# microsoft/SpeechT5

Hardware: AMD Instinct MI355X
Metric: audio-sec/s fwd+bwd SpeechT5-Base (higher is better)
Workload: dtype bf16

## Files before the change

### speecht5_amd/csrc/gemm.hip

```cpp
#include <type_traits>
#include "common.h"
#include "stream_scratch.h"
#include "../../include/speecht5_hip.h"

namespace {

constexpr int BM = 128, BN = 128, NTHREADS = 256;
constexpr int TILE_BYTES = 128 * 128;
constexpr int EP_LD = 68;

struct OpAddr {
  long long ld, bstride, seg_stride;
  int rpb, seg;
  __device__ __forceinline__ long long outer(int idx) const {
    return rpb ? (long long)(idx / rpb) * bstride + (long long)(idx % rpb) * ld : (long long)idx * ld;
  }
  __device__ __forceinline__ long long inner(int idx) const {
    return seg ? (long long)(idx / seg) * seg_stride + (idx % seg) : (long long)idx;
  }
};
__device__ __forceinline__ OpAddr make_addr(long long ld, long long bstride, long long seg_stride, int rpb, int seg) {
  OpAddr a; a.ld = ld; a.bstride = bstride; a.seg_stride = seg_stride; a.rpb = rpb; a.seg = seg;
  return a;
}
// ... 768 lines not shown
  if (p.dropout_p > 0.f) f |= F_DROP;
  if (p.R.ptr) f |= F_RES;
  if (p.Cpre.ptr) f |= F_PRE;
  if (p.beta != 0.f) f |= F_BETA;
  switch (f) {
    case 0: case F_GELU | F_PRE: case F_DROP | F_RES: case F_DACT: case F_BETA: case F_RES: return f;
    default: break;
  }
  if (log_rt) fprintf(stderr, "st5_gemm rt-epilogue feat=%d act=%d M=%d N=%d K=%d batch=%d\n", f, p.act, p.M, p.N, p.K, p.batch);
  return -1;
}

template <int... FS> struct FeatSet {};
typedef FeatSet<0, F_GELU | F_PRE, F_DROP | F_RES, F_DACT, F_BETA, F_RES> NtFeats;
typedef FeatSet<0, F_BETA> TnFeats;
template <int... FS, typename Fn>
int with_feat(const int feat, FeatSet<FS...>, Fn&& fn) {
  int rc = ST5_OK;
  const bool hit = ((feat == FS && (rc = fn(std::integral_constant<int, FS>()), true)) || ...);
  return hit ? rc : fn(std::integral_constant<int, -1>());
}
typedef __attribute__((address_space(3))) void* lds_ptr_t;
typedef const __attribute__((address_space(1))) void* gbl_ptr_t;

#ifndef GEMM_ABL
#define GEMM_ABL 0
#endif
#ifdef GEMM_TIMING
__device__ unsigned long long g_gemm_timing[8];
#define GPROBE(i) do { __builtin_amdgcn_s_waitcnt(0xC07F); const unsigned long long t_ = __builtin_amdgcn_s_memtime(); tacc[i] += (unsigned int)(t_ - tprev); tprev = t_; } while (0)
#else
#define GPROBE(i)
#endif

template <typename F, int OFF>
__device__ __forceinline__ F lds_read128_asm(const unsigned lds_addr) {
  static_assert(sizeof(F) == 16, "128-bit fragment");
  F v;
  asm volatile("ds_read_b128 %0, %1 offset:%2" : "=v"(v) : "v"(lds_addr), "n"(OFF) : "memory");
  return v;
}

#ifndef GLDS_AUX_A
#define GLDS_AUX_A 0
#endif
#ifndef GLDS_AUX_B
#define GLDS_AUX_B 0
#endif
template <typename T, int NBUF, int FEAT = -1>
__global__ __launch_bounds__(NTHREADS, 2) void gemm_nt_glds_kernel(const st5_gemm_params p, const int c_vec_ok) {
  if (st5_gate_dropped(p.gate)) return;
  ST5_PAD_TO_256_VGPRS();
#ifdef GEMM_TIMING
  unsigned int tacc[8] = {0, 0, 0, 0, 0, 0, 0, 0};
  unsigned long long tprev = __builtin_amdgcn_s_memtime();
#endif
  constexpr int VEC = Elem<T>::VEC;
  constexpr int BK = 128 / (int)sizeof(T);
  typedef typename Frag<T>::type frag_t;
  extern __shared__ __attribute__((aligned(16))) char dsm[];

  const int tid = threadIdx.x, lane = tid & 63, wave = tid >> 6;
  const int wr = wave >> 1, wc = wave & 1;
  const int z = blockIdx.z;
  const int tiles_n = (p.N + BN - 1) / BN;
// ... 3 lines not shown
  const int m0 = tm * BM, n0 = tn * BN;
  const T* Ap = reinterpret_cast<const T*>(p.A.ptr) + z_off(p.A.zs0, p.A.zs1, z, p.zdiv);
  const T* Bp = reinterpret_cast<const T*>(p.B.ptr) + z_off(p.B.zs0, p.B.zs1, z, p.zdiv);
  const OpAddr aa = make_addr(p.A.ld, p.A.bstride, 0, p.A.rpb, 0);
  const OpAddr ab = make_addr(p.B.ld, p.B.bstride, 0, p.B.rpb, 0);

  const T* asrc[4];
  const T* bsrc[4];
  const int rsub = lane >> 3, pc = lane & 7;
#pragma unroll
  for (int i = 0; i < 4; ++i) {
    const int row = (i * 4 + wave) * 8 + rsub;
    const int c = pc ^ ((row >> 1) & 7);
    int gr = m0 + row; gr = gr < p.M ? gr : p.M - 1;
    asrc[i] = Ap + aa.outer(gr) + c * VEC;
    int gc = n0 + row; gc = gc < p.N ? gc : p.N - 1;
    bsrc[i] = Bp + ab.outer(gc) + c * VEC;
  }
  const int dst0 = wave * 1024;

  auto issue = [&](int kt, int buf) {
    char* base = dsm + buf * 2 * TILE_BYTES + dst0;
#pragma unroll
    for (int i = 0; i < 4; ++i) {
      __builtin_amdgcn_global_load_lds((gbl_ptr_t)(asrc[i] + (long long)kt * BK), (lds_ptr_t)(base + i * 4096), 16, 0, GLDS_AUX_A);
      __builtin_amdgcn_global_load_lds((gbl_ptr_t)(bsrc[i] + (long long)kt * BK), (lds_ptr_t)(base + TILE_BYTES + i * 4096), 16, 0, GLDS_AUX_B);
    }
  };
  auto issue_a = [&](int kt, int slot) {
    char* base = dsm + slot * TILE_BYTES + dst0;
#pragma unroll
    for (int i = 0; i < 4; ++i)
      __builtin_amdgcn_global_load_lds((gbl_ptr_t)(asrc[i] + (long long)kt * BK), (lds_ptr_t)(base + i * 4096), 16, 0, GLDS_AUX_A);
  };
  auto issue_b = [&](int kt, int slot) {
    char* base = dsm + slot * TILE_BYTES + dst0;
#pragma unroll
    for (int i = 0; i < 4; ++i)
      __builtin_amdgcn_global_load_lds((gbl_ptr_t)(bsrc[i] + (long long)kt * BK), (lds_ptr_t)(base + i * 4096), 16, 0, GLDS_AUX_B);
  };

  f32x16 acc00, acc01, acc10, acc11;
#pragma unroll
  for (int r = 0; r < 16; ++r) { acc00[r] = 0.f; acc01[r] = 0.f; acc10[r] = 0.f; acc11[r] = 0.f; }

  const int nk = p.K / BK;
  if constexpr (NBUF == 5) {
    issue_a(0, 0); issue_b(0, 1);
    if (nk > 1) issue_a(1, 2);
  } else {
#pragma unroll
    for (int t = 0; t < NBUF - 1; ++t)
      if (t < nk) issue(t, t);
  }
  const int frow = lane & 31, fhalf = lane >> 5;
  const int arow0 = wr * 64 + frow, brow0 = wc * 64 + frow;
  const unsigned lds_base = (unsigned)(size_t)(lds_ptr_t)dsm;
  const unsigned a_addr0 = lds_off(arow0, fhalf), b_addr0 = lds_off(brow0, fhalf);
  GPROBE(0);
  int sa = 0;
  for (int kt = 0; kt < nk; ++kt) {
    if constexpr (NBUF == 5) {
      if (kt + 1 < nk) asm volatile("s_waitcnt vmcnt(4)" ::: "memory");
      else asm volatile("s_waitcnt vmcnt(0)" ::: "memory");
    } else {
      int ahead = nk - 1 - kt;
      ahead = ahead < NBUF - 2 ? ahead : NBUF - 2;
      if (ahead >= 3) asm volatile("s_waitcnt vmcnt(24)" ::: "memory");
      else if (ahead == 2) asm volatile("s_waitcnt vmcnt(16)" ::: "memory");
      else if (ahead == 1) asm volatile("s_waitcnt vmcnt(8)" ::: "memory");
      else asm volatile("s_waitcnt vmcnt(0)" ::: "memory");
    }
    __builtin_amdgcn_s_barrier();
    GPROBE(1);
#if GEMM_ABL != 2
    if constexpr (NBUF == 5) {
      if (kt + 1 < nk) issue_b(kt + 1, sa + 3 >= 5 ? sa - 2 : sa + 3);
      if (kt + 2 < nk) issue_a(kt + 2, sa + 4 >= 5 ? sa - 1 : sa + 4);
    } else {
      if (kt + NBUF - 1 < nk) issue(kt + NBUF - 1, (kt + NBUF - 1) % NBUF);
    }
#endif
    unsigned pa, pb;
    if constexpr (NBUF == 5) {
      const int sb = sa + 1 >= 5 ? 0 : sa + 1;
      pa = lds_base + sa * TILE_BYTES + a_addr0; pb = lds_base + sb * TILE_BYTES + b_addr0;
      sa = sa + 2 >= 5 ? sa - 3 : sa + 2;
    } else {
      const unsigned cb = lds_base + (kt % NBUF) * 2 * TILE_BYTES;
      pa = cb + a_addr0; pb = cb + TILE_BYTES + b_addr0;
    }
    frag_t fa0[2], fa1[2], fb0[2], fb1[2];
#define NT_READ(S, KG)                                                                                      \
  fa0[S] = lds_read128_asm<frag_t, 0>(pa ^ ((KG) << 5)); fb0[S] = lds_read128_asm<frag_t, 0>(pb ^ ((KG) << 5));          \
  fa1[S] = lds_read128_asm<frag_t, 4096>(pa ^ ((KG) << 5)); fb1[S] = lds_read128_asm<frag_t, 4096>(pb ^ ((KG) << 5));
#define NT_WAIT(S, CNT)                                                                                     \
  asm volatile("s_waitcnt lgkmcnt(" #CNT ")" : "+v"(fa0[S]), "+v"(fa1[S]), "+v"(fb0[S]), "+v"(fb1[S]) :: "memory");
#if GEMM_ABL == 3
#define NT_MMA(S) asm volatile("" :: "v"(fa0[S]), "v"(fa1[S]), "v"(fb0[S]), "v"(fb1[S]));
#else
#define NT_MMA(S)                                                                                           \
  mma<T>(fa0[S], fb0[S], acc00); mma<T>(fa0[S], fb1[S], acc01); mma<T>(fa1[S], fb0[S], acc10); mma<T>(fa1[S], fb1[S], acc11);
#endif
    NT_READ(0, 0)
    NT_READ(1, 1)
    NT_WAIT(0, 4)
    NT_MMA(0) __builtin_amdgcn_sched_barrier(0);
    NT_READ(0, 2)
    NT_WAIT(1, 4)
    NT_MMA(1) __builtin_amdgcn_sched_barrier(0);
    NT_READ(1, 3)
    NT_WAIT(0, 4)
// ... 32 lines not shown
  float* stage = reinterpret_cast<float*>(dsm) + wave * (32 * EP_LD);
#if GEMM_ABL == 1
  asm volatile("" :: "v"(acc00), "v"(acc01), "v"(acc10), "v"(acc11));
  if (ea.alpha == 123.f)
#endif
  run_epilogue<T, FEAT>(ea, stage, acc00, acc01, acc10, acc11, m0 + wr * 64, n0 + wc * 64, lane);
#ifdef GEMM_TIMING
  GPROBE(4);
  if (lane == 0) { for (int i = 0; i < 5; ++i) atomicAdd(&g_gemm_timing[i], (unsigned long long)tacc[i]); atomicAdd(&g_gemm_timing[7], 1ull); }
#endif
}


constexpr int M64_A_BYTES = 64 * 128, M64_STAGE = M64_A_BYTES + TILE_BYTES;

template <int FEAT>
__global__ __launch_bounds__(NTHREADS, 3) void gemm_nt_m64_kernel(const st5_gemm_params p, const int c_vec_ok) {
  if (st5_gate_dropped(p.gate)) return;
  typedef bf16_t T;
  constexpr int VEC = 8, BK = 64;
  typedef bf16x8 frag_t;
  extern __shared__ __attribute__((aligned(16))) char dsm[];

  const int tid = threadIdx.x, lane = tid & 63, wave = tid >> 6;
  const int wr = wave >> 1, wc = wave & 1;
  const int z = blockIdx.z;
  const int tiles_n = (p.N + BN - 1) / BN;
  const int bid = xcd_remap((int)blockIdx.x, (int)gridDim.x);
  int tm, tn;
  tile_of(bid, tiles_n, (int)gridDim.x, tm, tn);
  const int m0 = tm * 64, n0 = tn * BN;
// ... 1 lines not shown
  const T* Bp = reinterpret_cast<const T*>(p.B.ptr) + z_off(p.B.zs0, p.B.zs1, z, p.zdiv);
  const OpAddr aa = make_addr(p.A.ld, p.A.bstride, 0, p.A.rpb, 0);
  const OpAddr ab = make_addr(p.B.ld, p.B.bstride, 0, p.B.rpb, 0);

  const T* asrc[2];
  const T* bsrc[4];
  const int rsub = lane >> 3, pc = lane & 7;
#pragma unroll
  for (int i = 0; i < 4; ++i) {
    const int row = (i * 4 + wave) * 8 + rsub;
    const int c = pc ^ ((row >> 1) & 7);
    if (i < 2) {
      int gr = m0 + row; gr = gr < p.M ? gr : p.M - 1;
      asrc[i] = Ap + aa.outer(gr) + c * VEC;
    }
    int gc = n0 + row; gc = gc < p.N ? gc : p.N - 1;
    bsrc[i] = Bp + ab.outer(gc) + c * VEC;
  }
  const int dst0 = wave * 1024;
  auto issue = [&](int kt, int buf) {
    char* base = dsm + buf * M64_STAGE + dst0;
#pragma unroll
    for (int i = 0; i < 2; ++i)
      __builtin_amdgcn_global_load_lds((gbl_ptr_t)(asrc[i] + (long long)kt * BK), (lds_ptr_t)(base + i * 4096), 16, 0, 0);
#pragma unroll
    for (int i = 0; i < 4; ++i)
      __builtin_amdgcn_global_load_lds((gbl_ptr_t)(bsrc[i] + (long long)kt * BK), (lds_ptr_t)(base + M64_A_BYTES + i * 4096), 16, 0, 0);
  };

  f32x16 acc0, acc1;
#pragma unroll
  for (int r = 0; r < 16; ++r) { acc0[r] = 0.f; acc1[r] = 0.f; }

  const int nk = p.K / BK;
  issue(0, 0);
  const int frow = lane & 31, fhalf = lane >> 5;
  const unsigned lds_base = (unsigned)(size_t)(lds_ptr_t)dsm;
  const unsigned a_addr0 = lds_off(wr * 32 + frow, fhalf), b_addr0 = M64_A_BYTES + lds_off(wc * 64 + frow, fhalf);
  for (int kt = 0; kt < nk; ++kt) {
    asm volatile("s_waitcnt vmcnt(0)" ::: "memory");
    __builtin_amdgcn_s_barrier();
    if (kt + 1 < nk) issue(kt + 1, (kt + 1) & 1);
    const unsigned cb = lds_base + (kt & 1) * M64_STAGE;
    const unsigned pa = cb + a_addr0, pb = cb + b_addr0;
    frag_t fa[2], fb0[2], fb1[2];
#define M64_READ(S, KG)                                                                                     \
  fa[S] = lds_read128_asm<frag_t, 0>(pa ^ ((KG) << 5)); fb0[S] = lds_read128_asm<frag_t, 0>(pb ^ ((KG) << 5));           \
  fb1[S] = lds_read128_asm<frag_t, 4096>(pb ^ ((KG) << 5));
#define M64_WAIT(S, CNT)                                                                                    \
  asm volatile("s_waitcnt lgkmcnt(" #CNT ")" : "+v"(fa[S]), "+v"(fb0[S]), "+v"(fb1[S]) :: "memory");
#define M64_MMA(S) mma<T>(fa[S], fb0[S], acc0); mma<T>(fa[S], fb1[S], acc1);
    M64_READ(0, 0)
    M64_READ(1, 1)
    M64_WAIT(0, 3)
    M64_MMA(0) __builtin_amdgcn_sched_barrier(0);
    M64_READ(0, 2)
    M64_WAIT(1, 3)
    M64_MMA(1) __builtin_amdgcn_sched_barrier(0);
    M64_READ(1, 3)
    M64_WAIT(0, 3)
    M64_MMA(0) __builtin_amdgcn_sched_barrier(0);
    M64_WAIT(1, 0)
    M64_MMA(1) __builtin_amdgcn_sched_barrier(0);
#undef M64_READ
#undef M64_WAIT
// ... 190 lines not shown
      if (ea.out_f32) ea.R = reinterpret_cast<const float*>(ea.R) + zr; else ea.R = reinterpret_cast<const T*>(ea.R) + zr;
    }
    if (ea.P) ea.P = reinterpret_cast<const T*>(ea.P) + z_off(p.P.zs0, p.P.zs1, z, p.zdiv);
    if (ea.Cpre) ea.Cpre = reinterpret_cast<T*>(ea.Cpre) + z_off(p.Cpre.zs0, p.Cpre.zs1, z, p.zdiv);
  }
  float* stage = reinterpret_cast<float*>(dsm) + wave * (32 * EP_LD);
  run_epilogue<T>(ea, stage, acc[0][0], acc[0][1], acc[1][0], acc[1][1], m0 + wr * 128, n0 + wc * 64, lane);
  run_epilogue<T>(ea, stage, acc[2][0], acc[2][1], acc[3][0], acc[3][1], m0 + wr * 128 + 64, n0 + wc * 64, lane);
#ifdef GEMM_TIMING
  GPROBE(4);
  if (lane == 0) { for (int i = 0; i < 5; ++i) atomicAdd(&g_gemm_timing[i], (unsigned long long)tacc[i]); atomicAdd(&g_gemm_timing[7], 1ull); }
#endif
}


template <int FEAT, bool STAGGER>
__global__ __launch_bounds__(512) void gemm_nt8p_kernel(const st5_gemm_params p, const int c_vec_ok) {
  if (st5_gate_dropped(p.gate)) return;
  typedef bf16_t T;
  constexpr int BK = 64;
  constexpr int HALF = TILE_BYTES;
  constexpr int BUF = 4 * HALF;
  extern __shared__ __attribute__((aligned(16))) char dsm[];
  const int tid = threadIdx.x, lane = tid & 63;
  const int wave = __builtin_amdgcn_readfirstlane(tid >> 6);
  const int wr = wave >> 2, wc = wave & 3;
  const int z = blockIdx.z;
  const int tiles_n = (p.N + 255) / 256;
  const int bid = xcd_remap((int)blockIdx.x, (int)gridDim.x);
  int tm, tn;
  tile_of(bid, tiles_n, (int)gridDim.x, tm, tn);
// ... 2 lines not shown
  const T* Bp = reinterpret_cast<const T*>(p.B.ptr) + z_off(p.B.zs0, p.B.zs1, z, p.zdiv);
  const OpAddr aa = make_addr(p.A.ld, p.A.bstride, 0, p.A.rpb, 0);
  const OpAddr ab = make_addr(p.B.ld, p.B.bstride, 0, p.B.rpb, 0);

  const T* src[4][2];
  {
    const int rsub = lane >> 3, pc = lane & 7;
#pragma unroll
    for (int i = 0; i < 2; ++i) {
      const int row = (i * 8 + wave) * 8 + rsub;
      const int c = pc ^ ((row >> 1) & 7);
#pragma unroll
      for (int h = 0; h < 2; ++h) {
        int gr = m0 + h * 128 + row; gr = gr < p.M ? gr : p.M - 1;
        src[h][i] = Ap + aa.outer(gr) + c * 8;
        int gc = n0 + h * 128 + row; gc = gc < p.N ? gc : p.N - 1;
        src[2 + h][i] = Bp + ab.outer(gc) + c * 8;
      }
    }
  }
  auto stage = [&](const int h, const int kt) {
    char* base = dsm + (kt & 1) * BUF + h * HALF + wave * 1024;
#pragma unroll
    for (int i = 0; i < 2; ++i)
      __builtin_amdgcn_global_load_lds((gbl_ptr_t)(src[h][i] + (long long)kt * BK), (lds_ptr_t)(base + i * 8192), 16, 0, 0);
  };

  f32x16 acc[4][2];
#pragma unroll
  for (int i = 0; i < 4; ++i)
#pragma unroll
    for (int j = 0; j < 2; ++j)
#pragma unroll
      for (int r = 0; r < 16; ++r) acc[i][j][r] = 0.f;

  const int nk = p.K / BK;
  const int frow = lane & 31, fhalf = lane >> 5;
  int foff[4];
#pragma unroll
  for (int kg = 0; kg < 4; ++kg) foff[kg] = lds_off(frow, 2 * kg + fhalf);
  const int a_half = wr * HALF;
  const int b_base = (2 + (wc >> 1)) * HALF + (wc & 1) * 64 * 128;

  stage(0, 0); stage(1, 0); stage(2, 0); stage(3, 0);
  if (nk > 1) { stage(0, 1); stage(1, 1); asm volatile("s_waitcnt vmcnt(4)" ::: "memory"); }
  else asm volatile("s_waitcnt vmcnt(0)" ::: "memory");
  __builtin_amdgcn_s_barrier();
  if (STAGGER && wr == 1) __builtin_amdgcn_s_barrier();

  bf16x8 af[4][4], bfr[4];
  for (int t = 0; t < nk; ++t) {
    const char* cur = dsm + (t & 1) * BUF;
#pragma unroll
    for (int kg = 0; kg < 4; ++kg) bfr[kg] = *reinterpret_cast<const bf16x8*>(cur + b_base + foff[kg]);
    __builtin_amdgcn_sched_barrier(0);
#pragma unroll
    for (int i = 0; i < 4; ++i)
#pragma unroll
      for (int kg = 0; kg < 4; ++kg) af[i][kg] = *reinterpret_cast<const bf16x8*>(cur + a_half + i * 4096 + foff[kg]);
    if (t + 1 < nk) stage(2, t + 1);
    __builtin_amdgcn_s_barrier();
    asm volatile("s_waitcnt lgkmcnt(0)" ::: "memory");
    __builtin_amdgcn_sched_barrier(0);
    __builtin_amdgcn_s_setprio(1);
#pragma unroll
    for (int kg = 0; kg < 4; ++kg) { mma<T>(af[0][kg], bfr[kg], acc[0][0]); mma<T>(af[1][kg], bfr[kg], acc[1][0]); }
    __builtin_amdgcn_s_setprio(0);
    __builtin_amdgcn_s_barrier();
    if (t + 1 < nk) stage(3, t + 1);
    __builtin_amdgcn_s_barrier();
    __builtin_amdgcn_s_setprio(1);
#pragma unroll
    for (int kg = 0; kg < 4; ++kg) { mma<T>(af[2][kg], bfr[kg], acc[2][0]); mma<T>(af[3][kg], bfr[kg], acc[3][0]); }
    __builtin_amdgcn_s_setprio(0);
    __builtin_amdgcn_s_barrier();
#pragma unroll
    for (int kg = 0; kg < 4; ++kg) bfr[kg] = *reinterpret_cast<const bf16x8*>(cur + b_base + 4096 + foff[kg]);
    if (t + 2 < nk) stage(0, t + 2);
    __builtin_amdgcn_s_barrier();
    asm volatile("s_waitcnt lgkmcnt(0)" ::: "memory");
    __builtin_amdgcn_sched_barrier(0);
    __builtin_amdgcn_s_setprio(1);
#pragma unroll
    for (int kg = 0; kg < 4; ++kg) { mma<T>(af[2][kg], bfr[kg], acc[2][1]); mma<T>(af[3][kg], bfr[kg], acc[3][1]); }
    __builtin_amdgcn_s_setprio(0);
    __builtin_amdgcn_s_barrier();
    if (t + 2 < nk) { stage(1, t + 2); asm volatile("s_waitcnt vmcnt(4)" ::: "memory"); }
    else asm volatile("s_waitcnt vmcnt(0)" ::: "memory");
    __builtin_amdgcn_s_barrier();
    __builtin_amdgcn_s_setprio(1);
#pragma unroll
    for (int kg = 0; kg < 4; ++kg) { mma<T>(af[0][kg], bfr[kg], acc[0][1]); mma<T>(af[1][kg], bfr[kg], acc[1][1]); }
// ... 17 lines not shown
  {
    const long long zc = z_off(p.C.zs0, p.C.zs1, z, p.zdiv);
    if (ea.out_f32) ea.C = reinterpret_cast<float*>(ea.C) + zc; else ea.C = reinterpret_cast<T*>(ea.C) + zc;
    if (ea.R) {
      const long long zr = z_off(p.R.zs0, p.R.zs1, z, p.zdiv);
      if (ea.out_f32) ea.R = reinterpret_cast<const float*>(ea.R) + zr; else ea.R = reinterpret_cast<const T*>(ea.R) + zr;
    }
    if (ea.P) ea.P = reinterpret_cast<const T*>(ea.P) + z_off(p.P.zs0, p.P.zs1, z, p.zdiv);
    if (ea.Cpre) ea.Cpre = reinterpret_cast<T*>(ea.Cpre) + z_off(p.Cpre.zs0, p.Cpre.zs1, z, p.zdiv);
  }
  float* stg = reinterpret_cast<float*>(dsm) + wave * (32 * EP_LD);
  run_epilogue<T, FEAT>(ea, stg, acc[0][0], acc[0][1], acc[1][0], acc[1][1], m0 + wr * 128, n0 + wc * 64, lane);
  run_epilogue<T, FEAT>(ea, stg, acc[2][0], acc[2][1], acc[3][0], acc[3][1], m0 + wr * 128 + 64, n0 + wc * 64, lane);
}

int launch_nt8p(const st5_gemm_params& p, int c_vec_ok, bool stagger, hipStream_t s) {
  const int tiles = ((p.M + 255) / 256) * ((p.N + 255) / 256);
  const dim3 grid(tiles, 1, p.batch), block(512);
  const size_t lds = (size_t)8 * TILE_BYTES;
  return with_feat(nt_feat_of(p, c_vec_ok), NtFeats(), [&](auto f) -> int {
    constexpr int F = decltype(f)::value;
    return stagger ? launch_lds<gemm_nt8p_kernel<F, true>>(grid, block, lds, s, p, c_vec_ok)
                   : launch_lds<gemm_nt8p_kernel<F, false>>(grid, block, lds, s, p, c_vec_ok);
  });
}

template <typename T>
int launch_nt256(const st5_gemm_params& p, int c_vec_ok, hipStream_t s) {
  const int tiles = ((p.M + BM2 - 1) / BM2) * ((p.N + BN2 - 1) / BN2);
  return launch_lds<gemm_nt256_kernel<T>>(dim3(tiles, 1, p.batch), dim3(NT2), (size_t)NSTAGE2 * STAGE2_BYTES, s, p, c_vec_ok);
}

#ifdef GEMM_TIMING
}
extern "C" int st5_gemm_timing(unsigned long long* out, int reset) {
  if (hipMemcpyFromSymbol(out, HIP_SYMBOL(g_gemm_timing), sizeof(g_gemm_timing)) != hipSuccess) return ST5_ERR_LAUNCH;
  if (reset) { unsigned long long z[8] = {0, 0, 0, 0, 0, 0, 0, 0}; if (hipMemcpyToSymbol(HIP_SYMBOL(g_gemm_timing), z, sizeof(z)) != hipSuccess) return ST5_ERR_LAUNCH; }
  return ST5_OK;
}
namespace {
#endif


template <typename T, int NBUF>
int launch_glds_feat(const st5_gemm_params& p, int c_vec_ok, dim3 grid, hipStream_t s) {
  auto go = [&](auto f) -> int {
    return launch_lds<gemm_nt_glds_kernel<T, NBUF, decltype(f)::value>>(grid, dim3(NTHREADS), (size_t)(NBUF == 5 ? 5 : NBUF * 2) * TILE_BYTES, s, p, c_vec_ok);
  };
  if constexpr (sizeof(T) == 2) return with_feat(rt_epilogue_only() ? -1 : nt_feat_of(p, c_vec_ok), NtFeats(), go);
  else return go(std::integral_constant<int, -1>());
}

int launch_m64(const st5_gemm_params& p, int c_vec_ok, hipStream_t s) {
  const int tiles = ((p.M + 63) / 64) * ((p.N + BN - 1) / BN);
  const dim3 grid(tiles, 1, p.batch);
  return with_feat(nt_feat_of(p, c_vec_ok), NtFeats(), [&](auto f) -> int {
    return launch_lds<gemm_nt_m64_kernel<decltype(f)::value>>(grid, dim3(NTHREADS), (size_t)2 * M64_STAGE, s, p, c_vec_ok);
  });
}
bool nt_m64_pays(const st5_gemm_params& p) {
  static const int env = getenv("ST5_M64_MAX_TILES") ? atoi(getenv("ST5_M64_MAX_TILES")) : -1;
  const int lim = env >= 0 ? env : g_m64_max_tiles;
  const long long t128 = (long long)((p.M + BM - 1) / BM) * ((p.N + BN - 1) / BN) * p.batch;
  return t128 <= lim && p.M > 64;
}

template <typename T>
int launch_glds(const st5_gemm_params& p, int c_vec_ok, hipStream_t s) {
  const int tiles = ((p.M + BM - 1) / BM) * ((p.N + BN - 1) / BN);
  dim3 grid(tiles, 1, p.batch);
  const int nk = p.K / (128 / (int)sizeof(T));
  const bool deep = sizeof(T) == 2 && (long long)tiles * p.batch <= g_deep_blocks && nk >= 4 && g_deep_nbuf > 2;
  if constexpr (sizeof(T) == 2) {
    if (deep && g_deep_nbuf == 4) return launch_glds_feat<T, 4>(p, c_vec_ok, grid, s);
    if (deep) return launch_glds_feat<T, 3>(p, c_vec_ok, grid, s);
    if (g_nt_slots5 && nk >= 2) return launch_glds_feat<T, 5>(p, c_vec_ok, grid, s);
  }
  return launch_glds_feat<T, 2>(p, c_vec_ok, grid, s);
}

__device__ __attribute__((aligned(256))) char g_zero_page[256];
typedef __attribute__((ext_vector_type(4))) short s16x4;
typedef __attribute__((address_space(3))) s16x4* lds_s16x4_ptr;

__device__ __forceinline__ bf16x8 tr_frag(const char* tile_row, int off0, int off1) {
  const s16x4 lo = __builtin_amdgcn_ds_read_tr16_b64_v4i16((lds_s16x4_ptr)(tile_row + off0));
  const s16x4 hi = __builtin_amdgcn_ds_read_tr16_b64_v4i16((lds_s16x4_ptr)(tile_row + off1));
  union { struct { s16x4 a, b; } s; bf16x8 v; } u;
  u.s.a = lo; u.s.b = hi;
  return u.v;
}

template <int OFF>
__device__ __forceinline__ bf16x8 tr_frag_asm(const unsigned lds_addr) {
  s16x4 lo, hi;
  asm volatile("ds_read_b64_tr_b16 %0, %1 offset:%2" : "=v"(lo) : "v"(lds_addr), "n"(OFF) : "memory");
  asm volatile("ds_read_b64_tr_b16 %0, %1 offset:%2" : "=v"(hi) : "v"(lds_addr), "n"(OFF + 1024) : "memory");
  union { struct { s16x4 a, b; } s; bf16x8 v; } u;
  u.s.a = lo; u.s.b = hi;
  return u.v;
}

template <int FEAT>
__device__ __forceinline__ void tn_glds_body(const st5_gemm_params& p, const int c_vec_ok, const int bx, const int nwg_, const int by,
                                             const int ny, const int z, const bool remap = true) {
  typedef bf16_t T;
  constexpr int BK = 64;
  extern __shared__ __attribute__((aligned(16))) char dsm[];
  const int tid = threadIdx.x, lane = tid & 63, wave = tid >> 6;
  const int wr = wave >> 1, wc = wave & 1;
  const int tiles_n = (p.N + BN - 1) / BN;
  const int bid = remap ? xcd_remap(bx, nwg_) : bx;
// ... 843 lines not shown
    return ST5_OK;
  }
  const int bk = 128 / es;
  if (g_use_glds && !p.asum && !(p.flags & (ST5_GEMM_A_KSTRIDED | ST5_GEMM_B_KSTRIDED)) && p.K % bk == 0 && p.K >= 2 * bk && !p.A.seg && !p.B.seg)
  {
    if ((g_nt_tile == 3 || g_nt_tile == 4) && dtype == ST5_BF16 && p.K % 64 == 0) return launch_nt8p(p, c_vec_ok, g_nt_tile == 3, s);
    if (g_nt_tile == 2) return dtype == ST5_BF16 ? launch_nt256<bf16_t>(p, c_vec_ok, s) : launch_nt256<float>(p, c_vec_ok, s);
    if (g_nt_tile == 5 && dtype == ST5_BF16) return launch_m64(p, c_vec_ok, s);
    if (g_nt_tile == 0 && dtype == ST5_BF16 && nt_m64_pays(p) && !nt256_pays(p.M, p.N, p.K / 64, p.batch)) return launch_m64(p, c_vec_ok, s);
    if (g_nt_tile == 0 && nt256_pays(p.M, p.N, p.K / 64, p.batch)) {
      if (dtype == ST5_BF16 && p.K % 64 == 0) return launch_nt8p(p, c_vec_ok, true, s);
      if (dtype != ST5_BF16) return launch_nt256<float>(p, c_vec_ok, s);
    }
    return dtype == ST5_BF16 ? launch_glds<bf16_t>(p, c_vec_ok, s) : launch_glds<float>(p, c_vec_ok, s);
  }
  return launch_general(p, dtype, use8p, c_vec_ok, nsplit, s);
}

namespace {
bool tn_group_phased_shape(int M, int N, int K) { return g_tn_group_tile == 0 && M % 256 == 0 && N % 256 == 0 && K >= 512; }
bool tn_group_phased(const st5_gemm_params& p) {
  return tn_group_phased_shape(p.M, p.N, p.K) && p.C.ld % 4 == 0 && !p.A.rpb && !p.B.rpb && !p.A.seg && !p.B.seg;
}
}
extern "C" int st5_gemm_tn_group(const st5_gemm_params* list, int32_t n, int dtype, void* stream) {
  if (!list || n < 0) return ST5_ERR_ARG;
  hipStream_t s = reinterpret_cast<hipStream_t>(stream);
  TnGroupArgs g;
  Tn8pGroupArgs g8;
  int m = 0;
// ... 145 lines not shown
```

### speecht5_amd/ddp.py

```python
import contextlib
import os

import torch
import torch.distributed as dist

from . import functional as Fn



_SBS_STREAM_POOL = {}

class _Trigger(torch.autograd.Function):

    @staticmethod
    def forward(ctx, x, owner, bucket_id):
        ctx.owner, ctx.bucket_id = owner, bucket_id
        return x.view_as(x)

    @staticmethod
    def backward(ctx, g):
        ctx.owner._bucket_ready(ctx.bucket_id)
        return g, None, None


# ... 580 lines not shown
        self.lr, self.betas, self.eps, self.wd, self.clip = lr, betas, eps, weight_decay, clip_norm
        self.lr_step = None
        total = ddp.flat.numel()
        dev = ddp.flat.device
        self.pflat = torch.zeros(total, dtype=torch.float32, device=dev)
        offsets = list(ddp.offsets)
        for p, off in zip(ddp.params, offsets):
            n = p.numel()
            self.pflat[off:off + n].copy_(p.data.reshape(-1))
            p.data = self.pflat[off:off + n].view_as(p)
        self.mirror = None
        if dev.type == "cuda" and Fn._S.dtype == torch.bfloat16:
            self.wflat = self.pflat.to(torch.bfloat16)
            Fn.bf16_mirror.attach(self.wflat, ddp.params, offsets)
            cap = sum(p.numel() + 64 for p in ddp.params if p.dim() >= 2)
            Fn.bf16_mirror.tflat = torch.empty(cap, dtype=torch.bfloat16, device=dev)
            Fn.bf16_mirror.tcap = cap
            self.mirror = Fn.bf16_mirror
        self.m = torch.zeros_like(self.pflat)
        self.v = torch.zeros_like(self.pflat)
        self.gnorm_sq = torch.zeros(1, dtype=torch.float32, device=dev)
        self.t = 0
        self.guard = torch.zeros(GUARD_CELLS, dtype=torch.int32, device=dev) if skip_nonfinite else None
        self.hyper_dev = None
        self.hyper_host = None

    def enable_device_hyper(self):
        dev = self.pflat.device
        self.hyper_dev = torch.zeros(2, dtype=torch.float32, device=dev)
        self.hyper_host = torch.zeros(2, dtype=torch.float32).pin_memory()
        self.hyper_host2 = None
# ... 89 lines not shown
```

### speecht5_amd/functional.py

```python
import math
from types import SimpleNamespace

import os
import threading

import torch

from . import hip
from .hip import ACT_GELU, ACT_NONE, ACT_RELU, ACT_TANH

_S = SimpleNamespace(dtype=torch.float32, seed=0x5EED, counter=0, grad_hook=None, boundary_hook=None, side=None, side_raw=0,
                     side_keep=[], side_gens=[], side_n=0, attn_side=None, attn_side_raw=None, slots=None, force_static=False)


def set_compute_dtype(dtype):
    assert dtype in (torch.float32, torch.bfloat16)
    _S.dtype = dtype


def compute_dtype():
    return _S.dtype


def manual_seed(seed):
# ... 360 lines not shown
            self.waited.add(hip.stream())

    def transposed(self, off, rows, cols):
        self._sync_transposes()
        key = (off, rows, cols)
        hit = self.jobs.get(key)
        if hit is not None:
            ev = self.first.get(key)
            if ev is not None and ev[1] != hip.stream():
                torch.cuda.current_stream().wait_event(ev[0])
            return hit[1]
        n = rows * cols
        need = (self.tused + n + 63) // 64 * 64
        if need > self.tcap:
            return None
        view = self.tflat[self.tused:self.tused + n].view(cols, rows)
        self.jobs[key] = (self.tused, view)
        self.tused = need
        self.dirty = True
        _cast_free_transpose(self.flat[off:off + n].view(rows, cols), view)
        ev = torch.cuda.Event()
        ev.record()
        self.first[key] = (ev, hip.stream())
        return view

    def refresh_transposes(self):
        self.first = {}
        if not self.jobs:
            return
        if self.dirty or self.jobs_dev is None:
# ... 157 lines not shown
        _q8_tags[y.data_ptr()] = (y, q, sc, rows, cols)


def _q8_take(a2, rows, cols):
    with _q8_lock:
        hit = _q8_tags.pop(a2.data_ptr(), None)
    if hit is not None and hit[3:] == (rows, cols) and a2.is_contiguous():
        return hit[1], hit[2]
    return None


def _q8_buffers(rows, cols, device):
    return (torch.empty(rows, cols, dtype=torch.uint8, device=device), torch.empty(rows, cols // 32, dtype=torch.uint8, device=device))


def _nt_gemm(a2, weights, transposed, C, M, N, K, dtype, quant_out=None, **epi):
    W = fused_weight_t(weights, dtype) if transposed else fused_weight(weights, dtype)
    if _fp8_ok(M, N, K, dtype) and W.is_contiguous() and a2.is_contiguous():
        Wq, Ws = _quant_cached("qt" if transposed else "q", weights, W)
        pre = _q8_take(a2, M, K)
        aq, as_ = pre if pre is not None else hip.quant_mxfp8(a2)
        out_q = None
        if quant_out is not None and (_FP8.fuse & (4 if (epi.get("flags", 0) & hip.DACT) else 2)) and N % 128 == 0 and epi.get("dropout_p", 0.0) == 0 and epi.get("R") is None and \
                epi.get("beta", 0.0) == 0 and quant_out.is_contiguous() and quant_out.shape == (M, N) and \
                ((epi.get("flags", 0) & hip.DACT) or (epi.get("act", ACT_NONE) == ACT_GELU and epi.get("Cpre") is not None)):
            out_q = _q8_buffers(M, N, a2.device)
        hip.gemm_mxfp8(aq, as_, Wq, Ws, C, M, N, K, out_q=out_q, **epi)
        if out_q is not None:
            _q8_tag(quant_out, out_q[0], out_q[1], M, N)
        _FP8.launches += 1
        return
# ... 3043 lines not shown
```

Baseline: 3085.

## Add k-major B GEMM path using LDS transpose reads for dgrad

Adds a BNN template variant to the NT GEMM kernels (glds, m64, nt8p) in which B is loaded k-major straight from the untransposed weight mirror and transposed in LDS via ds_read_b64_tr_b16. The Python dgrad path now routes bf16 transposed-weight GEMMs through this path with a B_KSTRIDED flag, so the separate weight-transpose pass and its buffer are no longer needed. The transposed-weight buffer becomes lazily allocated. This trades a transpose kernel and its memory traffic for more complex LDS reads, changed lgkmcnt waits and an extra dispatch branch, which risks bank conflicts or lower MMA throughput.

```diff
diff --git a/speecht5_amd/csrc/gemm.hip b/speecht5_amd/csrc/gemm.hip
--- a/speecht5_amd/csrc/gemm.hip
+++ b/speecht5_amd/csrc/gemm.hip
@@ -806,6 +806,9 @@
 template <int... FS> struct FeatSet {};
 typedef FeatSet<0, F_GELU | F_PRE, F_DROP | F_RES, F_DACT, F_BETA, F_RES> NtFeats;
 typedef FeatSet<0, F_BETA> TnFeats;
+typedef FeatSet<0, F_DROP | F_RES, F_DACT, F_BETA, F_RES> NnFeats;
+template <bool BNN> struct NtFeatsOf { typedef NtFeats type; };
+template <> struct NtFeatsOf<true> { typedef NnFeats type; };
 template <int... FS, typename Fn>
 int with_feat(const int feat, FeatSet<FS...>, Fn&& fn) {
   int rc = ST5_OK;
@@ -833,14 +836,42 @@
   return v;
 }
 
+typedef __attribute__((ext_vector_type(4))) short s16x4;
+typedef __attribute__((address_space(3))) s16x4* lds_s16x4_ptr;
+
+template <int OFF>
+__device__ __forceinline__ bf16x8 tr_frag_asm(const unsigned lds_addr) {
+  s16x4 lo, hi;
+  asm volatile("ds_read_b64_tr_b16 %0, %1 offset:%2" : "=v"(lo) : "v"(lds_addr), "n"(OFF) : "memory");
+  asm volatile("ds_read_b64_tr_b16 %0, %1 offset:%2" : "=v"(hi) : "v"(lds_addr), "n"(OFF + 1024) : "memory");
+  union { struct { s16x4 a, b; } s; bf16x8 v; } u;
+  u.s.a = lo; u.s.b = hi;
+  return u.v;
+}
+
+__device__ __forceinline__ int tr_frag_off(const int lane, const int mbase) {
+  const int g = (lane >> 4) & 1, h = lane >> 5, j = (lane & 15) >> 2, q = lane & 3;
+  const int m = mbase + 16 * g + 4 * q;
+  const int pos = (m >> 3) ^ (4 * j);
+  return (8 * h + j) * 256 + pos * 16 + ((m >> 2) & 1) * 8;
+}
+
+__device__ __forceinline__ const bf16_t* nn_b_src(const bf16_t* Bp, const long long ldb, const int krow0, const int col0, const int N, const int lane) {
+  const int lrow = lane >> 4;
+  int col = col0 + (((lane & 15) ^ (4 * lrow)) << 3);
+  col = col < N ? col : N - 8;
+  return Bp + (long long)(krow0 + lrow) * ldb + col;
+}
+
 #ifndef GLDS_AUX_A
 #define GLDS_AUX_A 0
 #endif
 #ifndef GLDS_AUX_B
 #define GLDS_AUX_B 0
 #endif
-template <typename T, int NBUF, int FEAT = -1>
+template <typename T, int NBUF, int FEAT = -1, bool BNN = false>
 __global__ __launch_bounds__(NTHREADS, 2) void gemm_nt_glds_kernel(const st5_gemm_params p, const int c_vec_ok) {
+  static_assert(!BNN || sizeof(T) == 2, "B k-major form: bf16 only");
   if (st5_gate_dropped(p.gate)) return;
   ST5_PAD_TO_256_VGPRS();
 #ifdef GEMM_TIMING
@@ -874,17 +905,22 @@
     const int c = pc ^ ((row >> 1) & 7);
     int gr = m0 + row; gr = gr < p.M ? gr : p.M - 1;
     asrc[i] = Ap + aa.outer(gr) + c * VEC;
-    int gc = n0 + row; gc = gc < p.N ? gc : p.N - 1;
-    bsrc[i] = Bp + ab.outer(gc) + c * VEC;
+    if constexpr (BNN) {
+      bsrc[i] = nn_b_src(Bp, p.B.ld, (i * 4 + wave) * 4, n0, p.N, lane);
+    } else {
+      int gc = n0 + row; gc = gc < p.N ? gc : p.N - 1;
+      bsrc[i] = Bp + ab.outer(gc) + c * VEC;
+    }
   }
   const int dst0 = wave * 1024;
+  const long long bkstep = BNN ? (long long)BK * p.B.ld : (long long)BK;
 
   auto issue = [&](int kt, int buf) {
     char* base = dsm + buf * 2 * TILE_BYTES + dst0;
 #pragma unroll
     for (int i = 0; i < 4; ++i) {
       __builtin_amdgcn_global_load_lds((gbl_ptr_t)(asrc[i] + (long long)kt * BK), (lds_ptr_t)(base + i * 4096), 16, 0, GLDS_AUX_A);
-      __builtin_amdgcn_global_load_lds((gbl_ptr_t)(bsrc[i] + (long long)kt * BK), (lds_ptr_t)(base + TILE_BYTES + i * 4096), 16, 0, GLDS_AUX_B);
+      __builtin_amdgcn_global_load_lds((gbl_ptr_t)(bsrc[i] + kt * bkstep), (lds_ptr_t)(base + TILE_BYTES + i * 4096), 16, 0, GLDS_AUX_B);
     }
   };
   auto issue_a = [&](int kt, int slot) {
@@ -897,7 +933,7 @@
     char* base = dsm + slot * TILE_BYTES + dst0;
 #pragma unroll
     for (int i = 0; i < 4; ++i)
-      __builtin_amdgcn_global_load_lds((gbl_ptr_t)(bsrc[i] + (long long)kt * BK), (lds_ptr_t)(base + i * 4096), 16, 0, GLDS_AUX_B);
+      __builtin_amdgcn_global_load_lds((gbl_ptr_t)(bsrc[i] + kt * bkstep), (lds_ptr_t)(base + i * 4096), 16, 0, GLDS_AUX_B);
   };
 
   f32x16 acc00, acc01, acc10, acc11;
@@ -916,7 +952,8 @@
   const int frow = lane & 31, fhalf = lane >> 5;
   const int arow0 = wr * 64 + frow, brow0 = wc * 64 + frow;
   const unsigned lds_base = (unsigned)(size_t)(lds_ptr_t)dsm;
-  const unsigned a_addr0 = lds_off(arow0, fhalf), b_addr0 = lds_off(brow0, fhalf);
+  const unsigned a_addr0 = lds_off(arow0, fhalf), b_addr0 = BNN ? tr_frag_off(lane, wc * 64) : lds_off(brow0, fhalf);
+  const unsigned b_addr1 = BNN ? tr_frag_off(lane, wc * 64 + 32) : 0u;
   GPROBE(0);
   int sa = 0;
   for (int kt = 0; kt < nk; ++kt) {
@@ -941,21 +978,26 @@
       if (kt + NBUF - 1 < nk) issue(kt + NBUF - 1, (kt + NBUF - 1) % NBUF);
     }
 #endif
-    unsigned pa, pb;
+    unsigned pa, pb, pb1 = 0;
     if constexpr (NBUF == 5) {
       const int sb = sa + 1 >= 5 ? 0 : sa + 1;
       pa = lds_base + sa * TILE_BYTES + a_addr0; pb = lds_base + sb * TILE_BYTES + b_addr0;
+      if constexpr (BNN) pb1 = lds_base + sb * TILE_BYTES + b_addr1;
       sa = sa + 2 >= 5 ? sa - 3 : sa + 2;
     } else {
       const unsigned cb = lds_base + (kt % NBUF) * 2 * TILE_BYTES;
       pa = cb + a_addr0; pb = cb + TILE_BYTES + b_addr0;
+      if constexpr (BNN) pb1 = cb + TILE_BYTES + b_addr1;
     }
     frag_t fa0[2], fa1[2], fb0[2], fb1[2];
 #define NT_READ(S, KG)                                                                                      \
-  fa0[S] = lds_read128_asm<frag_t, 0>(pa ^ ((KG) << 5)); fb0[S] = lds_read128_asm<frag_t, 0>(pb ^ ((KG) << 5));          \
-  fa1[S] = lds_read128_asm<frag_t, 4096>(pa ^ ((KG) << 5)); fb1[S] = lds_read128_asm<frag_t, 4096>(pb ^ ((KG) << 5));
+  fa0[S] = lds_read128_asm<frag_t, 0>(pa ^ ((KG) << 5));                                                    \
+  if constexpr (BNN) fb0[S] = tr_frag_asm<(KG) * 4096>(pb); else fb0[S] = lds_read128_asm<frag_t, 0>(pb ^ ((KG) << 5));   \
+  fa1[S] = lds_read128_asm<frag_t, 4096>(pa ^ ((KG) << 5));                                                 \
+  if constexpr (BNN) fb1[S] = tr_frag_asm<(KG) * 4096>(pb1); else fb1[S] = lds_read128_asm<frag_t, 4096>(pb ^ ((KG) << 5));
 #define NT_WAIT(S, CNT)                                                                                     \
-  asm volatile("s_waitcnt lgkmcnt(" #CNT ")" : "+v"(fa0[S]), "+v"(fa1[S]), "+v"(fb0[S]), "+v"(fb1[S]) :: "memory");
+  if constexpr (BNN && CNT != 0) asm volatile("s_waitcnt lgkmcnt(6)" : "+v"(fa0[S]), "+v"(fa1[S]), "+v"(fb0[S]), "+v"(fb1[S]) :: "memory"); \
+  else asm volatile("s_waitcnt lgkmcnt(" #CNT ")" : "+v"(fa0[S]), "+v"(fa1[S]), "+v"(fb0[S]), "+v"(fb1[S]) :: "memory");
 #if GEMM_ABL == 3
 #define NT_MMA(S) asm volatile("" :: "v"(fa0[S]), "v"(fa1[S]), "v"(fb0[S]), "v"(fb1[S]));
 #else
@@ -1018,7 +1060,7 @@
 
 constexpr int M64_A_BYTES = 64 * 128, M64_STAGE = M64_A_BYTES + TILE_BYTES;
 
-template <int FEAT>
+template <int FEAT, bool BNN = false>
 __global__ __launch_bounds__(NTHREADS, 3) void gemm_nt_m64_kernel(const st5_gemm_params p, const int c_vec_ok) {
   if (st5_gate_dropped(p.gate)) return;
   typedef bf16_t T;
@@ -1050,10 +1092,15 @@
       int gr = m0 + row; gr = gr < p.M ? gr : p.M - 1;
       asrc[i] = Ap + aa.outer(gr) + c * VEC;
     }
-    int gc = n0 + row; gc = gc < p.N ? gc : p.N - 1;
-    bsrc[i] = Bp + ab.outer(gc) + c * VEC;
+    if constexpr (BNN) {
+      bsrc[i] = nn_b_src(Bp, p.B.ld, (i * 4 + wave) * 4, n0, p.N, lane);
+    } else {
+      int gc = n0 + row; gc = gc < p.N ? gc : p.N - 1;
+      bsrc[i] = Bp + ab.outer(gc) + c * VEC;
+    }
   }
   const int dst0 = wave * 1024;
+  const long long bkstep = BNN ? (long long)BK * p.B.ld : (long long)BK;
   auto issue = [&](int kt, int buf) {
     char* base = dsm + buf * M64_STAGE + dst0;
 #pragma unroll
@@ -1061,7 +1108,7 @@
       __builtin_amdgcn_global_load_lds((gbl_ptr_t)(asrc[i] + (long long)kt * BK), (lds_ptr_t)(base + i * 4096), 16, 0, 0);
 #pragma unroll
     for (int i = 0; i < 4; ++i)
-      __builtin_amdgcn_global_load_lds((gbl_ptr_t)(bsrc[i] + (long long)kt * BK), (lds_ptr_t)(base + M64_A_BYTES + i * 4096), 16, 0, 0);
+      __builtin_amdgcn_global_load_lds((gbl_ptr_t)(bsrc[i] + kt * bkstep), (lds_ptr_t)(base + M64_A_BYTES + i * 4096), 16, 0, 0);
   };
 
   f32x16 acc0, acc1;
@@ -1072,19 +1119,23 @@
   issue(0, 0);
   const int frow = lane & 31, fhalf = lane >> 5;
   const unsigned lds_base = (unsigned)(size_t)(lds_ptr_t)dsm;
-  const unsigned a_addr0 = lds_off(wr * 32 + frow, fhalf), b_addr0 = M64_A_BYTES + lds_off(wc * 64 + frow, fhalf);
+  const unsigned a_addr0 = lds_off(wr * 32 + frow, fhalf);
+  const unsigned b_addr0 = M64_A_BYTES + (BNN ? tr_frag_off(lane, wc * 64) : lds_off(wc * 64 + frow, fhalf));
+  const unsigned b_addr1 = BNN ? M64_A_BYTES + tr_frag_off(lane, wc * 64 + 32) : 0u;
   for (int kt = 0; kt < nk; ++kt) {
     asm volatile("s_waitcnt vmcnt(0)" ::: "memory");
     __builtin_amdgcn_s_barrier();
     if (kt + 1 < nk) issue(kt + 1, (kt + 1) & 1);
     const unsigned cb = lds_base + (kt & 1) * M64_STAGE;
-    const unsigned pa = cb + a_addr0, pb = cb + b_addr0;
+    const unsigned pa = cb + a_addr0, pb = cb + b_addr0, pb1 = cb + b_addr1;
     frag_t fa[2], fb0[2], fb1[2];
 #define M64_READ(S, KG)                                                                                     \
-  fa[S] = lds_read128_asm<frag_t, 0>(pa ^ ((KG) << 5)); fb0[S] = lds_read128_asm<frag_t, 0>(pb ^ ((KG) << 5));           \
-  fb1[S] = lds_read128_asm<frag_t, 4096>(pb ^ ((KG) << 5));
+  fa[S] = lds_read128_asm<frag_t, 0>(pa ^ ((KG) << 5));                                                     \
+  if constexpr (BNN) { fb0[S] = tr_frag_asm<(KG) * 4096>(pb); fb1[S] = tr_frag_asm<(KG) * 4096>(pb1); }     \
+  else { fb0[S] = lds_read128_asm<frag_t, 0>(pb ^ ((KG) << 5)); fb1[S] = lds_read128_asm<frag_t, 4096>(pb ^ ((KG) << 5)); }
 #define M64_WAIT(S, CNT)                                                                                    \
-  asm volatile("s_waitcnt lgkmcnt(" #CNT ")" : "+v"(fa[S]), "+v"(fb0[S]), "+v"(fb1[S]) :: "memory");
+  if constexpr (BNN && CNT != 0) asm volatile("s_waitcnt lgkmcnt(5)" : "+v"(fa[S]), "+v"(fb0[S]), "+v"(fb1[S]) :: "memory"); \
+  else asm volatile("s_waitcnt lgkmcnt(" #CNT ")" : "+v"(fa[S]), "+v"(fb0[S]), "+v"(fb1[S]) :: "memory");
 #define M64_MMA(S) mma<T>(fa[S], fb0[S], acc0); mma<T>(fa[S], fb1[S], acc1);
     M64_READ(0, 0)
     M64_READ(1, 1)
@@ -1305,7 +1356,7 @@
 }
 
 
-template <int FEAT, bool STAGGER>
+template <int FEAT, bool STAGGER, bool BNN = false>
 __global__ __launch_bounds__(512) void gemm_nt8p_kernel(const st5_gemm_params p, const int c_vec_ok) {
   if (st5_gate_dropped(p.gate)) return;
   typedef bf16_t T;
@@ -1338,16 +1389,21 @@
       for (int h = 0; h < 2; ++h) {
         int gr = m0 + h * 128 + row; gr = gr < p.M ? gr : p.M - 1;
         src[h][i] = Ap + aa.outer(gr) + c * 8;
-        int gc = n0 + h * 128 + row; gc = gc < p.N ? gc : p.N - 1;
-        src[2 + h][i] = Bp + ab.outer(gc) + c * 8;
+        if constexpr (BNN) {
+          src[2 + h][i] = nn_b_src(Bp, p.B.ld, (i * 8 + wave) * 4, n0 + h * 128, p.N, lane);
+        } else {
+          int gc = n0 + h * 128 + row; gc = gc < p.N ? gc : p.N - 1;
+          src[2 + h][i] = Bp + ab.outer(gc) + c * 8;
+        }
       }
     }
   }
+  const long long bkstep = BNN ? (long long)BK * p.B.ld : (long long)BK;
   auto stage = [&](const int h, const int kt) {
     char* base = dsm + (kt & 1) * BUF + h * HALF + wave * 1024;
 #pragma unroll
     for (int i = 0; i < 2; ++i)
-      __builtin_amdgcn_global_load_lds((gbl_ptr_t)(src[h][i] + (long long)kt * BK), (lds_ptr_t)(base + i * 8192), 16, 0, 0);
+      __builtin_amdgcn_global_load_lds((gbl_ptr_t)(src[h][i] + kt * (h < 2 ? (long long)BK : bkstep)), (lds_ptr_t)(base + i * 8192), 16, 0, 0);
   };
 
   f32x16 acc[4][2];
@@ -1365,6 +1421,9 @@
   for (int kg = 0; kg < 4; ++kg) foff[kg] = lds_off(frow, 2 * kg + fhalf);
   const int a_half = wr * HALF;
   const int b_base = (2 + (wc >> 1)) * HALF + (wc & 1) * 64 * 128;
+  const int boff0 = BNN ? (2 + (wc >> 1)) * HALF + tr_frag_off(lane, (wc & 1) * 64) : 0;
+  const int boff1 = BNN ? (2 + (wc >> 1)) * HALF + tr_frag_off(lane, (wc & 1) * 64 + 32) : 0;
+  const unsigned lds_base = (unsigned)(size_t)(lds_ptr_t)dsm;
 
   stage(0, 0); stage(1, 0); stage(2, 0); stage(3, 0);
   if (nk > 1) { stage(0, 1); stage(1, 1); asm volatile("s_waitcnt vmcnt(4)" ::: "memory"); }
@@ -1375,8 +1434,13 @@
   bf16x8 af[4][4], bfr[4];
   for (int t = 0; t < nk; ++t) {
     const char* cur = dsm + (t & 1) * BUF;
-#pragma unroll
-    for (int kg = 0; kg < 4; ++kg) bfr[kg] = *reinterpret_cast<const bf16x8*>(cur + b_base + foff[kg]);
+    if constexpr (BNN) {
+      const unsigned pb = lds_base + (t & 1) * BUF + boff0;
+      bfr[0] = tr_frag_asm<0>(pb); bfr[1] = tr_frag_asm<4096>(pb); bfr[2] = tr_frag_asm<8192>(pb); bfr[3] = tr_frag_asm<12288>(pb);
+    } else {
+#pragma unroll
+      for (int kg = 0; kg < 4; ++kg) bfr[kg] = *reinterpret_cast<const bf16x8*>(cur + b_base + foff[kg]);
+    }
     __builtin_amdgcn_sched_barrier(0);
 #pragma unroll
     for (int i = 0; i < 4; ++i)
@@ -1398,8 +1462,13 @@
     for (int kg = 0; kg < 4; ++kg) { mma<T>(af[2][kg], bfr[kg], acc[2][0]); mma<T>(af[3][kg], bfr[kg], acc[3][0]); }
     __builtin_amdgcn_s_setprio(0);
     __builtin_amdgcn_s_barrier();
-#pragma unroll
-    for (int kg = 0; kg < 4; ++kg) bfr[kg] = *reinterpret_cast<const bf16x8*>(cur + b_base + 4096 + foff[kg]);
+    if constexpr (BNN) {
+      const unsigned pb = lds_base + (t & 1) * BUF + boff1;
+      bfr[0] = tr_frag_asm<0>(pb); bfr[1] = tr_frag_asm<4096>(pb); bfr[2] = tr_frag_asm<8192>(pb); bfr[3] = tr_frag_asm<12288>(pb);
+    } else {
+#pragma unroll
+      for (int kg = 0; kg < 4; ++kg) bfr[kg] = *reinterpret_cast<const bf16x8*>(cur + b_base + 4096 + foff[kg]);
+    }
     if (t + 2 < nk) stage(0, t + 2);
     __builtin_amdgcn_s_barrier();
     asm volatile("s_waitcnt lgkmcnt(0)" ::: "memory");
@@ -1447,14 +1516,15 @@
   run_epilogue<T, FEAT>(ea, stg, acc[2][0], acc[2][1], acc[3][0], acc[3][1], m0 + wr * 128 + 64, n0 + wc * 64, lane);
 }
 
+template <bool BNN = false>
 int launch_nt8p(const st5_gemm_params& p, int c_vec_ok, bool stagger, hipStream_t s) {
   const int tiles = ((p.M + 255) / 256) * ((p.N + 255) / 256);
   const dim3 grid(tiles, 1, p.batch), block(512);
   const size_t lds = (size_t)8 * TILE_BYTES;
-  return with_feat(nt_feat_of(p, c_vec_ok), NtFeats(), [&](auto f) -> int {
+  return with_feat(nt_feat_of(p, c_vec_ok), typename NtFeatsOf<BNN>::type(), [&](auto f) -> int {
     constexpr int F = decltype(f)::value;
-    return stagger ? launch_lds<gemm_nt8p_kernel<F, true>>(grid, block, lds, s, p, c_vec_ok)
-                   : launch_lds<gemm_nt8p_kernel<F, false>>(grid, block, lds, s, p, c_vec_ok);
+    return stagger ? launch_lds<gemm_nt8p_kernel<F, true, BNN>>(grid, block, lds, s, p, c_vec_ok)
+                   : launch_lds<gemm_nt8p_kernel<F, false, BNN>>(grid, block, lds, s, p, c_vec_ok);
   });
 }
 
@@ -1475,20 +1545,21 @@
 #endif
 
 
-template <typename T, int NBUF>
+template <typename T, int NBUF, bool BNN = false>
 int launch_glds_feat(const st5_gemm_params& p, int c_vec_ok, dim3 grid, hipStream_t s) {
   auto go = [&](auto f) -> int {
-    return launch_lds<gemm_nt_glds_kernel<T, NBUF, decltype(f)::value>>(grid, dim3(NTHREADS), (size_t)(NBUF == 5 ? 5 : NBUF * 2) * TILE_BYTES, s, p, c_vec_ok);
+    return launch_lds<gemm_nt_glds_kernel<T, NBUF, decltype(f)::value, BNN>>(grid, dim3(NTHREADS), (size_t)(NBUF == 5 ? 5 : NBUF * 2) * TILE_BYTES, s, p, c_vec_ok);
   };
-  if constexpr (sizeof(T) == 2) return with_feat(rt_epilogue_only() ? -1 : nt_feat_of(p, c_vec_ok), NtFeats(), go);
+  if constexpr (sizeof(T) == 2) return with_feat(rt_epilogue_only() ? -1 : nt_feat_of(p, c_vec_ok), typename NtFeatsOf<BNN>::type(), go);
   else return go(std::integral_constant<int, -1>());
 }
 
+template <bool BNN = false>
 int launch_m64(const st5_gemm_params& p, int c_vec_ok, hipStream_t s) {
   const int tiles = ((p.M + 63) / 64) * ((p.N + BN - 1) / BN);
   const dim3 grid(tiles, 1, p.batch);
-  return with_feat(nt_feat_of(p, c_vec_ok), NtFeats(), [&](auto f) -> int {
-    return launch_lds<gemm_nt_m64_kernel<decltype(f)::value>>(grid, dim3(NTHREADS), (size_t)2 * M64_STAGE, s, p, c_vec_ok);
+  return with_feat(nt_feat_of(p, c_vec_ok), typename NtFeatsOf<BNN>::type(), [&](auto f) -> int {
+    return launch_lds<gemm_nt_m64_kernel<decltype(f)::value, BNN>>(grid, dim3(NTHREADS), (size_t)2 * M64_STAGE, s, p, c_vec_ok);
   });
 }
 bool nt_m64_pays(const st5_gemm_params& p) {
@@ -1498,37 +1569,24 @@
   return t128 <= lim && p.M > 64;
 }
 
-template <typename T>
+template <typename T, bool BNN = false>
 int launch_glds(const st5_gemm_params& p, int c_vec_ok, hipStream_t s) {
   const int tiles = ((p.M + BM - 1) / BM) * ((p.N + BN - 1) / BN);
   dim3 grid(tiles, 1, p.batch);
   const int nk = p.K / (128 / (int)sizeof(T));
   const bool deep = sizeof(T) == 2 && (long long)tiles * p.batch <= g_deep_blocks && nk >= 4 && g_deep_nbuf > 2;
   if constexpr (sizeof(T) == 2) {
-    if (deep && g_deep_nbuf == 4) return launch_glds_feat<T, 4>(p, c_vec_ok, grid, s);
-    if (deep) return launch_glds_feat<T, 3>(p, c_vec_ok, grid, s);
-    if (g_nt_slots5 && nk >= 2) return launch_glds_feat<T, 5>(p, c_vec_ok, grid, s);
-  }
-  return launch_glds_feat<T, 2>(p, c_vec_ok, grid, s);
+    if (deep && g_deep_nbuf == 4) return launch_glds_feat<T, 4, BNN>(p, c_vec_ok, grid, s);
+    if (deep) return launch_glds_feat<T, 3, BNN>(p, c_vec_ok, grid, s);
+    if (g_nt_slots5 && nk >= 2) return launch_glds_feat<T, 5, BNN>(p, c_vec_ok, grid, s);
+  }
+  return launch_glds_feat<T, 2, BNN>(p, c_vec_ok, grid, s);
 }
 
 __device__ __attribute__((aligned(256))) char g_zero_page[256];
-typedef __attribute__((ext_vector_type(4))) short s16x4;
-typedef __attribute__((address_space(3))) s16x4* lds_s16x4_ptr;
-
 __device__ __forceinline__ bf16x8 tr_frag(const char* tile_row, int off0, int off1) {
   const s16x4 lo = __builtin_amdgcn_ds_read_tr16_b64_v4i16((lds_s16x4_ptr)(tile_row + off0));
   const s16x4 hi = __builtin_amdgcn_ds_read_tr16_b64_v4i16((lds_s16x4_ptr)(tile_row + off1));
-  union { struct { s16x4 a, b; } s; bf16x8 v; } u;
-  u.s.a = lo; u.s.b = hi;
-  return u.v;
-}
-
-template <int OFF>
-__device__ __forceinline__ bf16x8 tr_frag_asm(const unsigned lds_addr) {
-  s16x4 lo, hi;
-  asm volatile("ds_read_b64_tr_b16 %0, %1 offset:%2" : "=v"(lo) : "v"(lds_addr), "n"(OFF) : "memory");
-  asm volatile("ds_read_b64_tr_b16 %0, %1 offset:%2" : "=v"(hi) : "v"(lds_addr), "n"(OFF + 1024) : "memory");
   union { struct { s16x4 a, b; } s; bf16x8 v; } u;
   u.s.a = lo; u.s.b = hi;
   return u.v;
@@ -2402,6 +2460,15 @@
     }
     return dtype == ST5_BF16 ? launch_glds<bf16_t>(p, c_vec_ok, s) : launch_glds<float>(p, c_vec_ok, s);
   }
+  if (g_use_glds && dtype == ST5_BF16 && p.batch == 1 && !p.asum && (p.flags & ST5_GEMM_B_KSTRIDED) && !(p.flags & ST5_GEMM_A_KSTRIDED) &&
+      !p.A.seg && !p.B.seg && !p.B.rpb && aligned(p.B.ptr, 16) && p.B.ld % 8 == 0 && p.N % 8 == 0 && p.K % 64 == 0 && p.K >= 128)
+  {
+    if (g_nt_tile == 3 || g_nt_tile == 4) return launch_nt8p<true>(p, c_vec_ok, g_nt_tile == 3, s);
+    if (g_nt_tile == 5) return launch_m64<true>(p, c_vec_ok, s);
+    if (g_nt_tile == 0 && nt_m64_pays(p) && !nt256_pays(p.M, p.N, p.K / 64, p.batch)) return launch_m64<true>(p, c_vec_ok, s);
+    if (g_nt_tile == 0 && nt256_pays(p.M, p.N, p.K / 64, p.batch)) return launch_nt8p<true>(p, c_vec_ok, true, s);
+    return launch_glds<bf16_t, true>(p, c_vec_ok, s);
+  }
   return launch_general(p, dtype, use8p, c_vec_ok, nsplit, s);
 }
 
diff --git a/speecht5_amd/ddp.py b/speecht5_amd/ddp.py
--- a/speecht5_amd/ddp.py
+++ b/speecht5_amd/ddp.py
@@ -618,7 +618,6 @@
             self.wflat = self.pflat.to(torch.bfloat16)
             Fn.bf16_mirror.attach(self.wflat, ddp.params, offsets)
             cap = sum(p.numel() + 64 for p in ddp.params if p.dim() >= 2)
-            Fn.bf16_mirror.tflat = torch.empty(cap, dtype=torch.bfloat16, device=dev)
             Fn.bf16_mirror.tcap = cap
             self.mirror = Fn.bf16_mirror
         self.m = torch.zeros_like(self.pflat)
diff --git a/speecht5_amd/functional.py b/speecht5_amd/functional.py
--- a/speecht5_amd/functional.py
+++ b/speecht5_amd/functional.py
@@ -398,6 +398,8 @@
         need = (self.tused + n + 63) // 64 * 64
         if need > self.tcap:
             return None
+        if self.tflat is None:
+            self.tflat = torch.empty(self.tcap, dtype=torch.bfloat16, device=self.flat.device)
         view = self.tflat[self.tused:self.tused + n].view(cols, rows)
         self.jobs[key] = (self.tused, view)
         self.tused = need
@@ -585,7 +587,17 @@
     return (torch.empty(rows, cols, dtype=torch.uint8, device=device), torch.empty(rows, cols // 32, dtype=torch.uint8, device=device))
 
 
+DGRAD_NN = os.environ.get("ST5_DGRAD_NN", "1") != "0"
+
+
 def _nt_gemm(a2, weights, transposed, C, M, N, K, dtype, quant_out=None, **epi):
+    if transposed and DGRAD_NN and dtype == torch.bfloat16 and N % 8 == 0 and not _fp8_ok(M, N, K, dtype):
+        hit = bf16_mirror.stacked(weights)
+        if hit is not None:
+            W = hit[1]
+            hip.gemm(hip.operand(a2, a2.stride(0)), hip.operand(W, W.shape[1]), C, M, N, K, _dt(dtype),
+                     **dict(epi, flags=epi.get("flags", 0) | hip.B_KSTRIDED))
+            return
     W = fused_weight_t(weights, dtype) if transposed else fused_weight(weights, dtype)
     if _fp8_ok(M, N, K, dtype) and W.is_contiguous() and a2.is_contiguous():
         Wq, Ws = _quant_cached("qt" if transposed else "q", weights, W)
```

Result: faster. 3122, median of 6 (+1.2%).
